# zju3dv/RelightableAvatar

Hardware: AMD Instinct MI355X
Metric: rays_per_sec (higher is better)
Workload: dtype f16

## Files before the change

### relightableavatar_amd/csrc/ra_api.cpp

```cpp
#include "ra_ctx.hpp"
#include <cmath>
#include <map>
#include <mutex>
#include <vector>

#include <cstring>
#include <cstdio>
#include <cstdlib>

static thread_local std::string g_err;
void ra_set_error(const std::string& msg) { g_err = msg; }

#define RA_CHECK(cond, msg)          \
    do {                             \
        if (!(cond)) {               \
            ra_set_error(msg);       \
            return 1;                \
        }                            \
    } while (0)

int DevBuf::ensure(size_t need) {
    if (need <= bytes && p) return 0;
    if (need == 0) need = 16;
    if (p) { hipDeviceSynchronize(); hipFree(p); p = nullptr; bytes = 0; }
// ... 313 lines not shown

void k3_launch(ra_ctx* c, const MlpIO& io, int n, hipStream_t s, int grid_slots = 0) {
    if (c->cfg.mlp_f16) launch_mlp_sdf_stream_f16(c->host.geo, c->sarena.p, c->sarena_pairs.p, c->barena.as<float>(), c->fr, io, n, s, grid_slots);
    else launch_mlp_sdf_stream_bf16(c->host.geo, c->sarena.p, c->sarena_pairs.p, c->barena.as<float>(), c->fr, io, n, s, grid_slots);
}

enum { Q_OTHER = 0, Q_SURFACE = 1 };
bool precise(const ra_ctx* c, int what) { return c->cfg.trace_precision >= 2 || (c->cfg.trace_precision == 1 && what == Q_SURFACE); }
constexpr int KEY_LIGHTS_MAX = 48;
bool key_tier(const ra_ctx* c) { return c->cfg.trace_precision == 1 && c->cfg.key_light_share > 0.f && c->n_lights > 0; }
int key_mask_from(ra_ctx* c, const float* probe, int ph, int pw, hipStream_t s) {
    if (c->key_external) return 0;
    c->key_valid = false;
    if (!key_tier(c) || !probe) return 0;
    if (c->key_mask.ensure((size_t)c->n_lights) || c->key_share.ensure((size_t)c->n_lights * sizeof(float))) return 1;
    launch_key_lights(probe, 1, ph, pw, c->light_dir.as<float>(), c->light_area.as<float>(), c->n_lights, c->cfg.key_light_share, KEY_LIGHTS_MAX, 0,
                      c->key_share.as<float>(), c->key_mask.as<unsigned char>(), s);
    c->key_valid = true;
    return 0;
}

void fine_level(ra_ctx* c, const MlpIO& io, int n, bool comp, hipStream_t s, int hint = -1) {
    const int nv = variant_size(n, hint);
    if (comp) {
        Timer t(c, s, 3);
        launch_mlp_sdf_comp(c->host.geo, c->sarena_c.p, c->barena.as<float>(), c->fr, io, nv, s, c->k3cc_ok, grid_size(n, nv));
    } else {
        Timer t(c, s, k3_waves(nv) == 8 ? 0 : 2);
        k3_launch(c, io, nv, s, grid_size(n, nv));
    }
}

int hdq_pass(ra_ctx* c, const RaySet& rs, int n, float th, int smooth, float* sdf, hipStream_t s, int what = Q_OTHER,
             const unsigned char* key = nullptr, int n_key = 0) {
    if (n <= 0) return 0;
    int err = 0;
    int* fine_idx = c->buf<int>("fine_idx", n, &err);
    float* bpts = c->buf<float>("fine_bpts", (size_t)n * 3, &err);
    if (err) return 1;
    HdqOut out{};
    out.sdf = sdf; out.fine_count = next_fine_counter(c, s); out.fine_idx = fine_idx; out.bpts = bpts;
    const int hint = fine_hint(c, c->fc_next - 1);
    int hint2 = -1;
    if (key && n_key > 0) {
        out.key = key;
        out.fine_idx2 = c->buf<int>("fine_idx_k", n_key, &err);
        out.bpts2 = c->buf<float>("fine_bpts_k", (size_t)n_key * 3, &err);
        if (err) return 1;
        out.fine_count2 = next_fine_counter(c, s);
        hint2 = fine_hint(c, c->fc_next - 1);
    }
    out.counters = dcnt(c);
    launch_hdq_coarse(c->fr, rs, n, th, c->cfg.blend_radius, out, s, c->cfg.use_geodesic_filter != 0);
    MlpIO io{};
    io.bpts = bpts; io.idx = fine_idx; io.count = out.fine_count; io.sdf = sdf; io.dist_th = th; io.smooth = smooth;
    io.resd_limit = c->cfg.resd_limit; io.counters = dcnt(c);
    fine_level(c, io, n, precise(c, what), s, hint);
    if (out.key) {
        io.bpts = out.bpts2; io.idx = out.fine_idx2; io.count = out.fine_count2;
        fine_level(c, io, n_key, true, s, hint2);
    }
    return 0;
}

int full_query(ra_ctx* c, FullIO io, int n, hipStream_t s) {
    const bool gated = c->gate && n > 65536;
    if (gated && c->gate->armed) RA_HIP(hipStreamWaitEvent(s, c->gate->done, 0));
    struct Release {
        ra_ctx* c; hipStream_t s; bool on;
        ~Release() { if (on) { hipEventRecord(c->gate->done, s); c->gate->armed = true; } }
    } release{c, s, gated};
    Timer t(c, s, 1);
    const int batch = c->cfg.k4_batch_slots > 0 ? c->cfg.k4_batch_slots : (1 << 20);
    const int cap = n < batch ? n : batch;
    int err = 0;
    char* tape = c->buf<char>("k4_tape", mlp_full_rev_tape_bytes(cap), &err);
    if (err) {
        ra_set_error("full query: no device memory for the activation tape (" + std::to_string(mlp_full_rev_tape_bytes(cap) >> 20) +
                     " MB): lower cfg.k4_batch_slots / cfg.volume_chunk_rays");
        return 1;
    }
    const bool f16w = c->cfg.mlp_f16 != 0;
    for (int s0 = 0; s0 < n; s0 += cap) {
        io.slot0 = s0;
        io.slot_cap = n - s0 < cap ? n - s0 : cap;
        if (f16w) {
// ... 189 lines not shown
    g.near_offset = near_offset; g.L = L; g.no_visibility = no_visibility; g.local_visibility = local_visibility;
    g.split_wide_groups = split_wide_groups ? 1 : 0;
    g.lvis = lvis; g.ldot = ldot;
    const bool traced = !(no_visibility || local_visibility);
    if (traced) {
        g.ray_pix = c->buf<int>("lv_pix", NR, &err);
        g.ray_light = c->buf<int>("lv_light", NR, &err);
        g.ray_slot = c->buf<int>("lv_slot", NR, &err);
        g.near_ = c->buf<float>("lv_near", NR, &err);
        g.far_ = c->buf<float>("lv_far", NR, &err);
    }
    g.ray_count = icnt(c, CNT_RAYS);
    TraceState sh{};
    float* ssdf = nullptr;
    if (traced) {
        sh = alloc_trace(c, "sh_", (int)NR, shadow.soft_shadow != 0, &err);
        ssdf = c->buf<float>("sh_sdf", NR, &err);
    }
    const bool keyed = traced && key_tier(c) && c->key_valid;
    const size_t NK = keyed ? (size_t)P * (size_t)(L < KEY_LIGHTS_MAX ? L : KEY_LIGHTS_MAX) : 0;
    if (err) return 1;
    if (c->gate && c->gate->armed) RA_HIP(hipStreamWaitEvent(s, c->gate->done, 0));
    launch_shadow_gen(g, P, s, c->cnt_zero);
    c->cnt_zero = false;
    if (traced) {
        sh.near_ = g.near_; sh.far_ = g.far_; sh.tan_i = c->light_sharp.as<float>(); sh.light = g.ray_light;
        launch_trace_init(sh, (int)NR, g.ray_count, shadow, s);
        RaySet r2{};
        r2.mode = 2; r2.o = surf; r2.t = sh.t; r2.pix = g.ray_pix; r2.light = g.ray_light; r2.ldir = c->light_dir.as<float>();
        r2.n_dev = g.ray_count;
        r2.skip = c->cfg.query_skip ? sh.stuck : nullptr;
        r2.nn_hint = c->buf<int>("lv_nn", NR * 3, &err);
        if (err) return 1;
        for (int it = 0; it < shadow.iters; ++it) {
            r2.hint_valid = it > 0;
            r2.hint_src = it == 0 ? pix_nn : nullptr;
            r2.hint_src_index = it == 0 ? g.ray_pix : nullptr;
            if (hdq_pass(c, r2, (int)NR, shadow.dist_th, 1, ssdf, s, Q_OTHER, keyed ? c->key_mask.as<unsigned char>() : nullptr, (int)NK)) return 1;
            launch_trace_update(sh, ssdf, (int)NR, g.ray_count, it, shadow, s);
        }
        launch_shadow_scatter(sh.occ, g.ray_slot, g.ray_count, (int)NR, lvis, s);
        launch_accumulate(g.ray_count, &dcnt(c)->n_shadow_rays, s);
    }
    if (c->gate) { RA_HIP(hipEventRecord(c->gate->done, s)); c->gate->armed = true; }
    *lvis_out = lvis;
    *ldot_out = ldot;
    return 0;
}

int ra_debug_key_lights(ra_ctx* c, unsigned char* key_dev, float* share_dev, void* stream) {
    RA_CHECK(c && key_dev && share_dev, "ra_debug_key_lights: null argument");
    RA_CHECK(c->key_valid && c->n_lights > 0, "ra_debug_key_lights: no key lights have been computed (ra_set_key_probes, or a render call with a probe)");
    RA_HIP(hipSetDevice(c->device));
    RA_HIP(hipMemcpyAsync(key_dev, c->key_mask.p, (size_t)c->n_lights, hipMemcpyDeviceToDevice, (hipStream_t)stream));
    RA_HIP(hipMemcpyAsync(share_dev, c->key_share.p, (size_t)c->n_lights * sizeof(float), hipMemcpyDeviceToDevice, (hipStream_t)stream));
    return 0;
}

int ra_begin_render(ra_ctx* c) {
    RA_CHECK(c, "ra_begin_render: null ctx");
    c->call_no = 0;
    return 0;
}

int ra_set_key_probes(ra_ctx* c, const float* probes, int n, int ph, int pw, int accumulate, void* stream) {
    RA_CHECK(c && n >= 0 && (n == 0 || (probes && ph > 0 && pw > 0)), "ra_set_key_probes: bad arguments");
    if (n == 0) { c->key_external = false; c->key_valid = false; return 0; }
    RA_CHECK(c->have_weights && c->n_lights > 0, "ra_set_key_probes: needs the relight network's light set (ra_finalize_weights)");
    RA_HIP(hipSetDevice(c->device));
    const bool acc = accumulate && c->key_external && c->key_valid;
    c->key_external = true;
    if (!key_tier(c)) { c->key_valid = false; return 0; }
    if (c->key_mask.ensure((size_t)c->n_lights) || c->key_share.ensure((size_t)c->n_lights * sizeof(float))) return 1;
    launch_key_lights(probes, n, ph, pw, c->light_dir.as<float>(), c->light_area.as<float>(), c->n_lights, c->cfg.key_light_share, KEY_LIGHTS_MAX,
// ... 759 lines not shown
```

### relightableavatar_amd/csrc/ra_hdq.hip

```cpp
#include "ra_kernels.hpp"
#include <type_traits>
#include <cstdlib>

namespace {

constexpr int KNN_THREADS = 256;

#ifdef RA_COARSE_TS
__device__ long long ra_coarse_ts[64 * 64 * 16 * 8];
extern "C" int ra_coarse_read_timestamps(long long* out) { return (int)hipMemcpyFromSymbol(out, HIP_SYMBOL(ra_coarse_ts), sizeof(ra_coarse_ts)); }
#define RA_CSTAMP(k) do { if (tsp) { __builtin_amdgcn_sched_barrier(0); if ((threadIdx.x & 63) == 0) tsp[k] = __builtin_readcyclecounter(); __builtin_amdgcn_sched_barrier(0); } } while (0)
#else
#define RA_CSTAMP(k) do { } while (0)
#endif
constexpr int VT = 2048;

__device__ __forceinline__ void inv3d(const float R[9], float M[9]) {
    M[0] = R[4] * R[8] - R[7] * R[5];
    M[3] = -R[3] * R[8] + R[6] * R[5];
    M[6] = R[3] * R[7] - R[6] * R[4];
    M[1] = -R[1] * R[8] + R[7] * R[2];
    M[4] = R[0] * R[8] - R[6] * R[2];
    M[7] = -R[0] * R[7] + R[6] * R[1];
    M[2] = R[1] * R[5] - R[4] * R[2];
    M[5] = -R[0] * R[5] + R[3] * R[2];
    M[8] = R[0] * R[4] - R[3] * R[1];
    const float D = R[0] * M[0] + R[1] * M[3] + R[2] * M[6];
    const float inv = 1.f / (D + 1e-8f);
#pragma unroll
    for (int i = 0; i < 9; ++i) M[i] *= inv;
}

__device__ __forceinline__ float sgn(float x) { return (x > 0.f) ? 1.f : ((x < 0.f) ? -1.f : 0.f); }
// ... 167 lines not shown
    }
}

template <int K>
__device__ __forceinline__ float row_bcast(float v) {
    return __int_as_float(__builtin_amdgcn_update_dpp(0, __float_as_int(v), 0x150 + K, 0xf, 0xf, false));
}

__device__ __forceinline__ float box_dist2(const float p[3], float lx, float ly, float lz, float hx, float hy, float hz) {
    const float dx = fmaxf(fmaxf(lx - p[0], p[0] - hx), 0.f);
    const float dy = fmaxf(fmaxf(ly - p[1], p[1] - hy), 0.f);
    const float dz = fmaxf(fmaxf(lz - p[2], p[2] - hz), 0.f);
    return dx * dx + dy * dy + dz * dz;
}

__device__ __forceinline__ float dist2(float dx, float dy, float dz) { return __fmaf_rn(dz, dz, __fmaf_rn(dx, dx, dy * dy)); }

__device__ __forceinline__ void knn_insert(float d, int id, float& d0, float& d1, float& d2, int& i0, int& i1, int& i2, bool dedup = false) {
    if (__builtin_expect(__ballot(d <= d2) == 0ull, 1)) return;
    bool fresh = true;
    if (dedup) fresh = (id != i0) & (id != i1) & (id != i2);
    const bool c2 = fresh && (d < d2 || (d == d2 && id < i2));
    const bool c1 = fresh && (d < d1 || (d == d1 && id < i1));
    const bool c0 = fresh && (d < d0 || (d == d0 && id < i0));
    const float nd2 = c1 ? d1 : (c2 ? d : d2);
    const int ni2 = c1 ? i1 : (c2 ? id : i2);
    const float nd1 = c0 ? d0 : (c1 ? d : d1);
    const int ni1 = c0 ? i0 : (c1 ? id : i1);
    d0 = c0 ? d : d0;
    i0 = c0 ? id : i0;
    d1 = nd1; i1 = ni1; d2 = nd2; i2 = ni2;
}

__device__ __forceinline__ void ray_point(const RaySet& rs, int i, float x[3]) {
    if (rs.mode == 0) {
        x[0] = rs.x[3 * i]; x[1] = rs.x[3 * i + 1]; x[2] = rs.x[3 * i + 2];
    } else if (rs.mode == 1) {
        const float t = rs.t[i];
        x[0] = rs.o[3 * i] + t * rs.d[3 * i];
        x[1] = rs.o[3 * i + 1] + t * rs.d[3 * i + 1];
        x[2] = rs.o[3 * i + 2] + t * rs.d[3 * i + 2];
    } else {
        const float t = rs.t[i];
        const int p = rs.pix[i], l = rs.light[i];
        x[0] = rs.o[3 * p] + t * rs.ldir[3 * l];
        x[1] = rs.o[3 * p + 1] + t * rs.ldir[3 * l + 1];
        x[2] = rs.o[3 * p + 2] + t * rs.ldir[3 * l + 2];
    }
}

template <bool BVH, int SPLIT, bool HINT = false>
__global__ __launch_bounds__(SPLIT == 1 ? KNN_THREADS : 64 * SPLIT) void hdq_coarse_kernel(FrameState fr, RaySet rs, int n_launch, float th, float inv2r2,
                                                                  HdqOut out, int dbg) {
    static_assert(SPLIT == 1 || (BVH && SPLIT >= 2 && SPLIT <= 16), "SPLIT > 1: the workgroup is SPLIT waves on the same 64 queries");
    constexpr int NT = SPLIT == 1 ? KNN_THREADS : 64 * SPLIT;
    __shared__ __attribute__((aligned(16))) unsigned char smem[BVH ? 16 : VT * 16];
#ifdef RA_COARSE_TS
    long long* tsp = blockIdx.x < 64 ? ra_coarse_ts + ((((dbg >> 8) & 63) * 64 + blockIdx.x) * 16 + (threadIdx.x >> 6)) * 8 : nullptr;
    dbg &= 255;
    if (tsp && (threadIdx.x & 63) == 0) { tsp[1] = tsp[2] = tsp[3] = tsp[4] = tsp[5] = tsp[6] = tsp[7] = 0; }
    RA_CSTAMP(0);
#endif
    const int n = rs.n_dev ? min(*rs.n_dev, n_launch) : n_launch;
    const int base = blockIdx.x * (SPLIT == 1 ? KNN_THREADS : 64);
    if (base >= n) return;
    if (blockIdx.x == 0 && threadIdx.x == 0 && out.counters) atomicAdd(&out.counters->n_coarse, (unsigned long long)n);
    const int i = base + (SPLIT == 1 ? threadIdx.x : (threadIdx.x & 63));
    const bool live_q = i < n && !(rs.skip && rs.skip[i < n ? i : 0]);
    bool live = live_q;
    if (__syncthreads_count(live_q) == 0) return;
    float x[3] = {0.f, 0.f, 0.f};
    if (live) ray_point(rs, i, x);
    const float xt[3] = {x[0] - fr.Th[0], x[1] - fr.Th[1], x[2] - fr.Th[2]};
    float p[3];
#pragma unroll
    for (int c = 0; c < 3; ++c) p[c] = xt[0] * fr.R[c] + xt[1] * fr.R[3 + c] + xt[2] * fr.R[6 + c];

    RA_CSTAMP(1);
    float d0 = 3.0e38f, d1 = 3.0e38f, d2 = 3.0e38f;
    int i0 = 0, i1 = 0, i2 = 0;
    if (dbg & 1) { d0 = 1e-4f; d1 = 2e-4f; d2 = 3e-4f; i0 = 0; i1 = 1; i2 = 2; }
    else if (BVH) {
        const int nl = fr.bvh_leaves, ns = fr.bvh_supers;
        if (!live) { d0 = d1 = d2 = -1.f; }
        const unsigned long long lm = __ballot(live);
        const int first = lm ? __ffsll((long long)lm) - 1 : 0;
        const int lane = threadIdx.x & 63;
        typedef float f2 __attribute__((ext_vector_type(2)));
        const f2 px2 = {p[0], p[0]}, py2 = {p[1], p[1]}, pz2 = {p[2], p[2]};
        constexpr bool hinted = HINT;
#ifdef RA_COARSE_TS
        int n_rare = 0;
#endif
        typedef float f8 __attribute__((ext_vector_type(8)));
        typedef float f4 __attribute__((ext_vector_type(4)));
        typedef int i4 __attribute__((ext_vector_type(4)));
        auto soa8 = [&](int off) __attribute__((always_inline)) { return *(const f8 __attribute__((address_space(4)))*)(fr.bvh_soa + off); };
        auto soa_id4 = [&](int off) __attribute__((always_inline)) { return *(const i4 __attribute__((address_space(4)))*)(fr.bvh_soa + off); };
        auto box4 = [&](int off) __attribute__((always_inline)) {
            return *(const f4 __attribute__((address_space(4)))*)(reinterpret_cast<const float*>(fr.bvh_sbox) + off);
        };
        auto box1 = [&](int off) __attribute__((always_inline)) { return reinterpret_cast<const float*>(fr.bvh_sbox)[off]; };
        auto scan_leaf = [&](int l) __attribute__((always_inline)) {
            const int L = l * (4 * BVH_LEAF);
            f8 cx = soa8(L), cy = soa8(L + BVH_LEAF), cz = soa8(L + 2 * BVH_LEAF), nx = cx, ny = cy, nz = cz;
// ... 242 lines not shown
#pragma unroll
        for (int e = 0; e < 24; ++e) out.dbg_mats[(size_t)i * 24 + e] = M[e];
    }
}

}

void launch_vert_blend(const float* weights, const float* A, const float* big_A, int n_verts, int n_bones, float* vertA,
                       hipStream_t s) {
    hipLaunchKernelGGL(vert_blend_kernel, dim3((n_verts + 255) / 256), dim3(256), 0, s, weights, A, big_A, n_verts, n_bones, vertA);
}

void launch_pack_verts(const float* pverts, int n_verts, float4* out, hipStream_t s) {
    hipLaunchKernelGGL(pack_verts_kernel, dim3((n_verts + 255) / 256), dim3(256), 0, s, pverts, n_verts, out);
}

void launch_fold_bias(const float* W, int ld, int col0, int ncond, const float* cond, const float* bias, float* out,
                      hipStream_t s) {
    hipLaunchKernelGGL(fold_bias_kernel, dim3(64), dim3(256), 0, s, W, ld, col0, ncond, cond, bias, out);
}

int bvh_leaf_count(int n_verts) {
    if (n_verts > BVH_MAXN) return 0;
    return (n_verts + BVH_LEAF - 1) / BVH_LEAF;
}
int bvh_super_count(int n_leaves) { return (n_leaves + BVH_FAN - 1) / BVH_FAN; }

void launch_bvh_build(const float4* pverts4, int n_verts, int* order, float* leaves, float4* sbox, int n_leaves, int n_supers, hipStream_t s) {
    hipLaunchKernelGGL(bvh_rank_kernel, dim3((n_verts + 63) / 64), dim3(BVH_THREADS), 0, s, pverts4, n_verts, order);
    hipLaunchKernelGGL(bvh_boxes_kernel, dim3(1), dim3(BVH_THREADS), 0, s, pverts4, order, n_verts, leaves, sbox, n_leaves, n_supers);
}

void launch_hdq_coarse(const FrameState& fr, const RaySet& rs, int n, float th, float blend_radius, const HdqOut& out,
                       hipStream_t s, bool geodesic) {
    if (n <= 0) return;
    const float inv2r2 = 1.f / (2.f * blend_radius * blend_radius);
    const dim3 grid((n + KNN_THREADS - 1) / KNN_THREADS);
    int dbg = 0, probe = 0, split_max = 196608;
#ifdef RA_TESTING
    static const int e_dbg = getenv("RA_COARSE_DBG") ? atoi(getenv("RA_COARSE_DBG")) : 0;
    static const int e_probe = getenv("RA_COARSE_PROBE") ? atoi(getenv("RA_COARSE_PROBE")) : 0;
    static const int e_split = getenv("RA_COARSE_SPLIT_MAX") ? atoi(getenv("RA_COARSE_SPLIT_MAX")) : 196608;
    dbg = e_dbg; probe = e_probe; split_max = e_split;
#endif
    if (!geodesic) dbg |= 32;
#ifdef RA_COARSE_TS
    static int launch_no = 0;
    dbg |= (launch_no++ & 63) << 8;
#endif
    const bool hint = (rs.nn_hint != nullptr && rs.hint_valid != 0) || rs.hint_src != nullptr;
    for (int pass = probe ? 0 : 1; pass < 2; ++pass) {
        const int d = pass == 0 ? probe : dbg;
        if (fr.bvh_leaves > 0 && n <= split_max)
        {
            const int groups = (n + 63) / 64;
            if (hint) {
                if (n <= split_max / 8) hipLaunchKernelGGL((hdq_coarse_kernel<true, 16, true>), dim3(groups), dim3(1024), 0, s, fr, rs, n, th, inv2r2, out, d);
                else if (n <= split_max / 2) hipLaunchKernelGGL((hdq_coarse_kernel<true, 8, true>), dim3(groups), dim3(512), 0, s, fr, rs, n, th, inv2r2, out, d);
                else hipLaunchKernelGGL((hdq_coarse_kernel<true, 4, true>), dim3(groups), dim3(256), 0, s, fr, rs, n, th, inv2r2, out, d);
            } else {
                if (n <= split_max / 8) hipLaunchKernelGGL((hdq_coarse_kernel<true, 16>), dim3(groups), dim3(1024), 0, s, fr, rs, n, th, inv2r2, out, d);
                else if (n <= split_max / 2) hipLaunchKernelGGL((hdq_coarse_kernel<true, 8>), dim3(groups), dim3(512), 0, s, fr, rs, n, th, inv2r2, out, d);
                else hipLaunchKernelGGL((hdq_coarse_kernel<true, 4>), dim3(groups), dim3(256), 0, s, fr, rs, n, th, inv2r2, out, d);
            }
        }
        else if (fr.bvh_leaves > 0 && hint) hipLaunchKernelGGL((hdq_coarse_kernel<true, 1, true>), grid, dim3(KNN_THREADS), 0, s, fr, rs, n, th, inv2r2, out, d);
        else if (fr.bvh_leaves > 0) hipLaunchKernelGGL((hdq_coarse_kernel<true, 1>), grid, dim3(KNN_THREADS), 0, s, fr, rs, n, th, inv2r2, out, d);
        else hipLaunchKernelGGL((hdq_coarse_kernel<false, 1>), grid, dim3(KNN_THREADS), 0, s, fr, rs, n, th, inv2r2, out, d);
        if (pass == 0) hipMemsetAsync(out.fine_count, 0, sizeof(int), s);
    }
}
```

### relightableavatar_amd/csrc/ra_kernels.hpp

```cpp
#pragma once
#include "ra_common.hpp"

struct RaySet {
    int mode;
    const float* x;
    const float* o;
    const float* d;
    const float* t;
    const int* pix;
    const int* light;
    const float* ldir;
    const int* n_dev;
    const unsigned char* skip;
    int* nn_hint;
    int hint_valid;
    const int* hint_src;
    const int* hint_src_index;
};

struct HdqOut {
    float* sdf;
    int* fine_count;
    int* fine_idx;
    float* bpts;
    float* mats;
    const unsigned char* key;
    int* fine_count2;
    int* fine_idx2;
    float* bpts2;
    float* raw_zero;
    int raw_C;
    float* dbg_sdf_batch;
    int* dbg_nn_batch;
    float* dbg_d2;
    float* dbg_tpts;
    float* dbg_bpts;
    float* dbg_mats;
    DevCounters* counters;
};

void launch_vert_blend(const float* weights, const float* A, const float* big_A, int n_verts, int n_bones, float* vertA,
                       hipStream_t s);
void launch_pack_verts(const float* pverts, int n_verts, float4* out, hipStream_t s);
void launch_fold_bias(const float* W, int ld, int col0, int ncond, const float* cond, const float* bias, float* out,
                      hipStream_t s);
void launch_bvh_build(const float4* pverts4, int n_verts, int* order, float* leaves, float4* sbox, int n_leaves, int n_supers, hipStream_t s);
int bvh_leaf_count(int n_verts);
int bvh_super_count(int n_leaves);
void launch_hdq_coarse(const FrameState& fr, const RaySet& rs, int n, float th, float blend_radius, const HdqOut& out,
                       hipStream_t s, bool geodesic = true);

struct TraceState {
    float *t, *d0, *dt, *st, *ot, *cd, *occ, *off, *rlx;
    const float *near_, *far_;
    const float* tan_i;
    const int* light;
    unsigned char* stuck;
};
void launch_trace_init(const TraceState& ts, int n, const int* n_dev, const ra_trace_params& p, hipStream_t s);

void launch_trace_update(const TraceState& ts, const float* sdf, int n, const int* n_dev, int iter,
                         const ra_trace_params& p, hipStream_t s);

void launch_surface_finish(const float* ray_o, const float* ray_d, const float* st, const float* occ, int P, float* surf,
                           float* depth, float* acc, int* hit_idx, int* hit_count, hipStream_t s, int* slot_of_ray = nullptr,
                           bool counter_is_zero = false);
void launch_slot_index(const int* hit_idx, const int* hit_count, int P, int* slot_of_ray, hipStream_t s);
struct MapJob { const float* src; float* dst; int C; int premul; int src_full; };
constexpr int RA_MAX_MAP_JOBS = 16;
struct EmitMaps { MapJob job[RA_MAX_MAP_JOBS]; long long end[RA_MAX_MAP_JOBS]; int n_jobs; const int* slot_of_ray; const float* acc; const int* perm; int P; };
void launch_emit_maps(const EmitMaps& m, hipStream_t s);
void launch_surface_samples(const float* surf, const float* ray_d, const int* hit_idx, const int* hit_count, int P, int S,
                            float range, float* x, float* v, int* n_out, hipStream_t s);
struct SurfaceMaps {
    float *cpts, *bpts, *resd, *norm, *albedo, *rough, *rgb;
    float* valbedo;
};
void launch_surface_composite(const float* raw, int C, int S, const int* hit_count, int P, int relight, const ra_config& cfg,
                              const SurfaceMaps& m, hipStream_t s);

constexpr int RA_MAX_BOXES = 32;
struct ShadowGen {
    const float* surf;
    const float* norm;
    const float* acc;
    const int* hit_idx;
    const int* hit_count;
    const float* ldir;
    float bbox[6];
    int n_boxes;
    float boxes[RA_MAX_BOXES][6];
    int box_start[RA_MAX_BOXES + 1];
    const int* perm;
    float near_offset;
    int L;
    int no_visibility, local_visibility;
    int split_wide_groups;
    float* lvis;
    float* ldot;
    int* ray_pix;
    int* ray_light;
    int* ray_slot;
    float *near_, *far_;
    int* ray_count;
};
void launch_key_lights(const float* probes, int n, int ph, int pw, const float* ldir, const float* area, int L, float share, int kmax,
                       int accumulate, float* smax, unsigned char* key, hipStream_t s);
void launch_gather_shard_rays(const long long* idx, int n, const float* ro, const float* rd, const float* nr, const float* fr, float* so, float* sd,
                              float* sn, float* sf, hipStream_t s);
void launch_scatter_rows(const float* src, const long long* src_idx, const long long* dst_idx, long long n, int C, float* dst, hipStream_t s);
void launch_shadow_gen(const ShadowGen& g, int P, hipStream_t s, bool counter_is_zero = false);
void launch_debug_aabb(const float* o, const float* d, int n, const float* bbox6, float* nr, float* fr, hipStream_t s);
void launch_debug_brdf(const float* p2l, const float* p2c, const float* nrm, const float* alb, const float* rough, int L, int N, const ra_config& cfg,
                       float* out, hipStream_t s);
size_t sort_hits_temp_bytes(int P);
int launch_sort_hits(const float* surf, const float* acc, int P, const float* bbox_min, unsigned* keys_in, unsigned* keys_out,
                     int* vals_in, int* hit_idx_out, void* temp, size_t temp_bytes, hipStream_t s);
void launch_shadow_scatter(const float* occ, const int* ray_slot, const int* ray_count, int max_rays, float* lvis, hipStream_t s);

struct ShadeIn {
    const float* ray_o;
    const float* surf;
    const int* idx;
    const int* count;
    int n;
    const float *norm, *albedo, *rough;
    const float *lvis, *ldot;
    const float *light_xyz, *light_area;
    int L;
    const float* probes;
    int n_probes, ph, pw;
    int want_spec;
    float *rgb, *shade, *spec;
};
void launch_shade(const ShadeIn& in, const ra_config& cfg, hipStream_t s);

void launch_scatter_maps(const int* hit_idx, const int* hit_count, int P, int premultiply, const float* acc_full,
                         const float* src, int C, float* dst, int src_full, const int* perm, hipStream_t s);
int launch_sort_rays(const float* ro, const float* rd, const float* nr, const float* fr, int P, const float* bbox_min, unsigned* keys_in,
                     unsigned* keys_out, int* vals_in, int* perm, void* temp, size_t temp_bytes, float* so, float* sd, float* sn, float* sf,
                     hipStream_t s, float near_min = -3.0e38f, float far_max = 3.0e38f);
void launch_accumulate(const int* count, unsigned long long* dst, hipStream_t s);

void launch_volume_samples(const float* ray_o, const float* ray_d, const float* near_, const float* far_, int P, int S,
                           float* x, float* v, hipStream_t s);
void launch_volume_composite(const float* raw, int C, const float* near_, const float* far_, int P, int S, float bg,
                             const ra_render_out& out, const int* perm, hipStream_t s);
void launch_fill(float* p, size_t n, float v, hipStream_t s);
void launch_iota(int* idx, int n, int* count, hipStream_t s);
void launch_bigpose_compose(const float* mats, const float* d2, int n, float blend_radius, const float* R, const float* Th, int invert, float* out,
                            hipStream_t s);
// ... 67 lines not shown
```

### relightableavatar_amd/csrc/ra_trace.hip

```cpp
#include "ra_kernels.hpp"
#include <hipcub/hipcub.hpp>

namespace {

constexpr int TPB = 256;
constexpr float PI_F = 3.14159265358979323846f;

__device__ __forceinline__ int live_count(const int* n_dev, int n) { return n_dev ? min(*n_dev, n) : n; }

__device__ __forceinline__ float linspace01(int s, int S) {
    if (S == 1) return 0.f;
    const float step = 1.f / (float)(S - 1);
    return (s < S / 2) ? (float)s * step : 1.f - (float)(S - 1 - s) * step;
}

__global__ void trace_init_kernel(TraceState ts, int n_launch, const int* n_dev, float offset, float relax) {
    const int i = blockIdx.x * TPB + threadIdx.x;
    if (i >= live_count(n_dev, n_launch)) return;
    const float nr = ts.near_[i], fr = ts.far_[i];
    ts.t[i] = nr;
    ts.d0[i] = 1e9f;
    ts.occ[i] = 1.f;
    if (ts.stuck) ts.stuck[i] = 0;
    if (ts.dt) ts.dt[i] = 1e9f;
    if (ts.st) ts.st[i] = fr;
    if (ts.ot) ts.ot[i] = fr;
    if (ts.cd) ts.cd[i] = 1e9f;
    if (ts.off) ts.off[i] = offset;
    if (ts.rlx) ts.rlx[i] = relax;
}

template <bool SOFT>
__global__ void trace_update_kernel(TraceState ts, const float* __restrict__ sdf, int n_launch, const int* n_dev, int iter,
                                    ra_trace_params p) {
    const int i = blockIdx.x * TPB + threadIdx.x;
    if (i >= live_count(n_dev, n_launch)) return;
    const float d1 = sdf[i];
    const float d0 = ts.d0[i];
    float t = ts.t[i];
    const float t_prev = t;
    float occ = ts.occ[i];
    const float nr = ts.near_[i], fr = ts.far_[i];
    float tan_i = p.tan_i;
    if (SOFT) {
        const float ti = ts.tan_i ? (ts.light ? ts.tan_i[ts.light[i]] : ts.tan_i[i]) : p.tan_i;
        tan_i = p.tan_i_multiplier * ti;
    }
    const float tan2 = (1.f / tan_i) * 2.f;
    float off = ts.off ? ts.off[i] : p.offset;
    float rlx = ts.rlx ? ts.rlx[i] : p.relax;
    float ot = ts.ot ? ts.ot[i] : 0.f;
    if (SOFT && p.clay_book && iter >= p.shadow_skip_iter) {
        const float dx0 = d0 + rlx * d0 + off;
        const float dx1 = d1 + rlx * d1 + off;
        const float dy = (dx1 * dx1) / (2.f * dx0);
        const float dx = (sqrtf(dx1 * dx1 - dy * dy) - off) / (1.f + rlx);
        const float den = fmaxf(fmaxf(t - dy, nr), p.eps);
        const float cls = fmaxf(dx, 0.f) / den / tan2;
        const bool msk = (cls < occ) && (dy < t) && (dx1 > 0.f) && (dx0 > 0.f) && (dx > 0.f) && (dy > 0.f) && (dy < dx0);
        if (msk) { ot = t - dy; occ = cls; }
    }
    if (iter >= p.shadow_skip_iter) {
        const float cls = fmaxf(d1, 0.f) / fmaxf(fmaxf(t, nr), p.eps) / tan2;
        if (cls < occ) { ot = t; occ = cls; }
    }
    if (!SOFT) {
        const float d1u = fabsf(d1), d0u = fabsf(d0);
        float st = ts.st[i], cd = ts.cd[i];
        const float dt = ts.dt[i];
        const float s0 = (d0 > 0.f) ? 1.f : ((d0 < 0.f) ? -1.f : 0.f);
        const float s1 = (d1 > 0.f) ? 1.f : ((d1 < 0.f) ? -1.f : 0.f);
        if (s0 != s1) {
            st = t - dt * fminf(fmaxf(d1u / (d0u + d1u + p.eps), 0.f), 1.f);
            off = 0.f;
            rlx = 0.f;
        }
        if (d1u < cd) { cd = d1u; st = t; }
        ts.st[i] = st;
        ts.cd[i] = cd;
        ts.off[i] = off;
        ts.rlx[i] = rlx;
    }
    const float dtn = d1 + rlx * d1 + off;
    t = t + dtn;
    t = fminf(t, fr);
    t = fmaxf(t, nr);
    if (ts.dt) ts.dt[i] = dtn;
    ts.t[i] = t;
    if (ts.stuck) ts.stuck[i] = (t == t_prev || (SOFT && occ == 0.f)) ? 1 : 0;
    ts.d0[i] = d1;
    ts.occ[i] = occ;
    if (ts.ot) ts.ot[i] = ot;
}

__global__ void surface_finish_kernel(const float* __restrict__ ro, const float* __restrict__ rd, const float* __restrict__ st,
                                      const float* __restrict__ occ, int P, float* __restrict__ surf, float* __restrict__ depth,
                                      float* __restrict__ acc, int* __restrict__ hit_idx, int* __restrict__ hit_count, int* __restrict__ slot_of_ray) {
    const int i = blockIdx.x * TPB + threadIdx.x;
    bool hit = false;
    if (i < P) {
        if (slot_of_ray) slot_of_ray[i] = -1;
        const float s = st[i];
        const float sx = ro[3 * i] + s * rd[3 * i], sy = ro[3 * i + 1] + s * rd[3 * i + 1], sz = ro[3 * i + 2] + s * rd[3 * i + 2];
        surf[3 * i] = sx; surf[3 * i + 1] = sy; surf[3 * i + 2] = sz;
        depth[i] = (sx - ro[3 * i]) / rd[3 * i];
        const float a = 1.f - occ[i];
        acc[i] = a;
        hit = a > 0.f;
    }
    const unsigned long long m = __ballot(hit);
    if (m == 0ull) return;
    const int lane = threadIdx.x & 63;
    int base = 0;
    if (lane == 0) base = atomicAdd(hit_count, __popcll(m));
    base = __shfl(base, 0);
    if (hit) hit_idx[base + __popcll(m & ((1ull << lane) - 1ull))] = i;
}

__device__ __forceinline__ unsigned expand10t(unsigned v) {
    v = (v * 0x00010001u) & 0xFF0000FFu;
    v = (v * 0x00000101u) & 0x0F00F00Fu;
    v = (v * 0x00000011u) & 0xC30C30C3u;
    v = (v * 0x00000005u) & 0x49249249u;
    return v;
}
// ... 268 lines not shown
    const int gbase = cnt[0][NL];
#pragma unroll
    for (int round = 0; round < ROUNDS; ++round) {
        const int ll = round * (TPB / 64) + wv;
        const bool trace = (tmask >> round) & 1u;
        const unsigned long long m = __ballot(trace);
        if (trace) {
            const int hf = lane >> 5;
            const unsigned mh = hf ? (unsigned)(m >> 32) : (unsigned)m;
            const int s = gbase + cnt[hf][ll] + __popc(mh & ((1u << (lane & 31)) - 1u));
            const int l = lc * SG_LIGHTS + ll;
            g.ray_pix[s] = r;
            g.ray_light[s] = l;
            g.ray_slot[s] = h * g.L + l;
            g.near_[s] = nrv[round];
            g.far_[s] = frv[round];
        }
    }
    const int col = threadIdx.x & (SG_LIGHTS - 1), l = lc * SG_LIGHTS + col;
    for (int row = threadIdx.x / SG_LIGHTS; row < 64; row += TPB / SG_LIGHTS) {
        const int hh = grp * 64 + row;
        if (hh < nh && l < g.L) {
            g.ldot[(size_t)hh * g.L + l] = t_ldot[row][col];
            g.lvis[(size_t)hh * g.L + l] = t_lvis[row][col];
        }
    }
}

__global__ void shadow_scatter_kernel(const float* __restrict__ occ, const int* __restrict__ ray_slot, const int* __restrict__ ray_count,
                                      int max_rays, float* __restrict__ lvis) {
    const int i = blockIdx.x * TPB + threadIdx.x;
    if (i >= min(*ray_count, max_rays)) return;
    lvis[ray_slot[i]] = occ[i];
}

__device__ __forceinline__ float safe_div(float& a, float& b) {
    const float eps = 1e-8f;
    if (a < eps && a >= 0.f) a = eps;
    if (a > -eps && a <= 0.f) a = -eps;
    if (b < eps && b >= 0.f) b = eps;
    if (b > -eps && b <= 0.f) b = -eps;
    float d = a / b;
    if (d != d) d = 0.f;
    if (isinf(d)) d = 0.f;
    return fminf(fmaxf(d, -1e10f), 1e10f);
}

__device__ __forceinline__ void fnormalize(float v[3]) {
    const float n = fmaxf(sqrtf(v[0] * v[0] + v[1] * v[1] + v[2] * v[2]), 1e-7f);
    v[0] /= n; v[1] /= n; v[2] /= n;
}

__device__ __forceinline__ void sample_probe(const float* __restrict__ img, int H, int W, const float d[3], float out[3]) {
    const float theta = acosf(d[2]) - 1e-6f;
    const float phi = atan2f(d[1], d[0]);
    const float qy = (theta / PI_F) * 2.f - 1.f;
    const float qx = -phi / PI_F;
    float ix = ((qx + 1.f) * W - 1.f) * 0.5f;
    float iy = ((qy + 1.f) * H - 1.f) * 0.5f;
    ix = fminf(fmaxf(ix, 0.f), (float)(W - 1));
    iy = fminf(fmaxf(iy, 0.f), (float)(H - 1));
    const float fx = floorf(ix), fy = floorf(iy);
    const int x0 = (int)fx, y0 = (int)fy, x1 = x0 + 1, y1 = y0 + 1;
    const float wx1 = ix - fx, wy1 = iy - fy, wx0 = 1.f - wx1, wy0 = 1.f - wy1;
    out[0] = out[1] = out[2] = 0.f;
    auto add = [&](int xx, int yy, float w) {
// ... 850 lines not shown
    size_t bytes = 0;
    hipcub::DeviceSelect::Flagged(nullptr, bytes, hipcub::CountingInputIterator<int>(0), (const unsigned char*)nullptr, (int*)nullptr, (int*)nullptr, n);
    return bytes;
}

int launch_gen_rays(const RayCam& cam, unsigned char* mask, int* pix_idx, int* count_dev, void* temp, size_t temp_bytes,
                    float* ray_o, float* ray_d, float* near, float* far, hipStream_t s) {
    const int n = cam.H * cam.W;
    if (n <= 0) { hipMemsetAsync(count_dev, 0, sizeof(int), s); return 0; }
    hipLaunchKernelGGL(ray_mask_kernel, grid_for(n), dim3(TPB), 0, s, cam, mask);
    if (hipcub::DeviceSelect::Flagged(temp, temp_bytes, hipcub::CountingInputIterator<int>(0), mask, pix_idx, count_dev, n, s) != hipSuccess) return 1;
    hipLaunchKernelGGL(ray_emit_kernel, grid_for(n), dim3(TPB), 0, s, cam, pix_idx, count_dev, ray_o, ray_d, near, far);
    return 0;
}

size_t sort_hits_temp_bytes(int P) {
    size_t bytes = 0;
    hipcub::DeviceRadixSort::SortPairs(nullptr, bytes, (const unsigned*)nullptr, (unsigned*)nullptr, (const int*)nullptr, (int*)nullptr, P);
    return bytes;
}

int launch_sort_hits(const float* surf, const float* acc, int P, const float* bbox_min, unsigned* keys_in, unsigned* keys_out,
                     int* vals_in, int* hit_idx_out, void* temp, size_t temp_bytes, hipStream_t s) {
    if (P <= 0) return 0;
    hipLaunchKernelGGL(hit_keys_kernel, grid_for(P), dim3(TPB), 0, s, surf, acc, P, bbox_min[0], bbox_min[1], bbox_min[2], keys_in, vals_in);
    return hipcub::DeviceRadixSort::SortPairs(temp, temp_bytes, keys_in, keys_out, vals_in, hit_idx_out, P, 0, 32, s) == hipSuccess ? 0 : 1;
}

void launch_shadow_scatter(const float* occ, const int* ray_slot, const int* ray_count, int max_rays, float* lvis, hipStream_t s) {
    if (max_rays <= 0) return;
    hipLaunchKernelGGL(shadow_scatter_kernel, grid_for(max_rays), dim3(TPB), 0, s, occ, ray_slot, ray_count, max_rays, lvis);
}

void launch_shade(const ShadeIn& in, const ra_config& cfg, hipStream_t s) {
    if (in.n <= 0) return;
    hipLaunchKernelGGL(shade_kernel, grid_for((long long)in.n * 64), dim3(TPB), 0, s, in, cfg);
}

void launch_scatter_maps(const int* hit_idx, const int* hit_count, int P, int premultiply, const float* acc_full, const float* src,
                         int C, float* dst, int src_full, const int* perm, hipStream_t s) {
    if (P <= 0) return;
    hipLaunchKernelGGL(scatter_maps_kernel, grid_for((long long)P * C), dim3(TPB), 0, s, hit_idx, hit_count, premultiply, acc_full, src, C, dst, src_full, perm);
}

int launch_sort_rays(const float* ro, const float* rd, const float* nr, const float* fr, int P, const float* bbox_min, unsigned* keys_in,
                     unsigned* keys_out, int* vals_in, int* perm, void* temp, size_t temp_bytes, float* so, float* sd, float* sn, float* sf,
                     hipStream_t s, float near_min, float far_max) {
    if (P <= 0) return 0;
    float* origin_dev = nullptr;
    if (!bbox_min) {
        origin_dev = reinterpret_cast<float*>(keys_out);
        hipLaunchKernelGGL(entry_min_kernel, dim3(1), dim3(1024), 0, s, ro, rd, nr, P, origin_dev);
    }
    hipLaunchKernelGGL(ray_keys_kernel, grid_for(P), dim3(TPB), 0, s, ro, rd, nr, P, bbox_min ? bbox_min[0] : 0.f, bbox_min ? bbox_min[1] : 0.f,
                       bbox_min ? bbox_min[2] : 0.f, origin_dev, keys_in, vals_in);
    if (hipcub::DeviceRadixSort::SortPairs(temp, temp_bytes, keys_in, keys_out, vals_in, perm, P, 0, 32, s) != hipSuccess) return 1;
    hipLaunchKernelGGL(gather_rays_kernel, grid_for(P), dim3(TPB), 0, s, perm, P, ro, rd, nr, fr, so, sd, sn, sf, near_min, far_max);
    return 0;
}

void launch_gather_shard_rays(const long long* idx, int n, const float* ro, const float* rd, const float* nr, const float* fr, float* so, float* sd,
                              float* sn, float* sf, hipStream_t s) {
    if (n <= 0) return;
    hipLaunchKernelGGL(gather_shard_rays_kernel, grid_for(n), dim3(TPB), 0, s, idx, n, ro, rd, nr, fr, so, sd, sn, sf);
}

// ... 90 lines not shown
```

Baseline: 9.017 million.

## Fuse soft-shadow trace update into next hdq coarse kernel and final scatter

For soft shadows, the per-iteration trace_update kernel is folded into the following hinted BVH coarse query kernel: each thread computes the trace step in registers, stores the state, and uses the new t directly for its ray point. The last iteration's update is merged into a new shadow_finish kernel that writes lvis directly. This removes one launch and one global round-trip of the trace state per iteration. In exchange there are more kernel template variants, more registers in the coarse kernel, and a fallback path when the BVH/hint conditions are not met.

```diff
diff --git a/relightableavatar_amd/csrc/ra_api.cpp b/relightableavatar_amd/csrc/ra_api.cpp
--- a/relightableavatar_amd/csrc/ra_api.cpp
+++ b/relightableavatar_amd/csrc/ra_api.cpp
@@ -369,7 +369,7 @@
 }
 
 int hdq_pass(ra_ctx* c, const RaySet& rs, int n, float th, int smooth, float* sdf, hipStream_t s, int what = Q_OTHER,
-             const unsigned char* key = nullptr, int n_key = 0) {
+             const unsigned char* key = nullptr, int n_key = 0, const TraceFuse* fuse = nullptr) {
     if (n <= 0) return 0;
     int err = 0;
     int* fine_idx = c->buf<int>("fine_idx", n, &err);
@@ -388,7 +388,7 @@
         hint2 = fine_hint(c, c->fc_next - 1);
     }
     out.counters = dcnt(c);
-    launch_hdq_coarse(c->fr, rs, n, th, c->cfg.blend_radius, out, s, c->cfg.use_geodesic_filter != 0);
+    launch_hdq_coarse(c->fr, rs, n, th, c->cfg.blend_radius, out, s, c->cfg.use_geodesic_filter != 0, fuse);
     MlpIO io{};
     io.bpts = bpts; io.idx = fine_idx; io.count = out.fine_count; io.sdf = sdf; io.dist_th = th; io.smooth = smooth;
     io.resd_limit = c->cfg.resd_limit; io.counters = dcnt(c);
@@ -644,14 +644,21 @@
         r2.skip = c->cfg.query_skip ? sh.stuck : nullptr;
         r2.nn_hint = c->buf<int>("lv_nn", NR * 3, &err);
         if (err) return 1;
+        static const bool fuse_env = !(getenv("RA_SHADOW_UPDATE_FUSED") && atoi(getenv("RA_SHADOW_UPDATE_FUSED")) == 0);
+        const bool fused = fuse_env && shadow.soft_shadow != 0 && shadow.iters > 0;
+        TraceFuse fu{};
+        fu.ts = sh; fu.sdf = ssdf; fu.p = shadow;
         for (int it = 0; it < shadow.iters; ++it) {
             r2.hint_valid = it > 0;
             r2.hint_src = it == 0 ? pix_nn : nullptr;
             r2.hint_src_index = it == 0 ? g.ray_pix : nullptr;
-            if (hdq_pass(c, r2, (int)NR, shadow.dist_th, 1, ssdf, s, Q_OTHER, keyed ? c->key_mask.as<unsigned char>() : nullptr, (int)NK)) return 1;
-            launch_trace_update(sh, ssdf, (int)NR, g.ray_count, it, shadow, s);
+            fu.iter = it - 1;
+            if (hdq_pass(c, r2, (int)NR, shadow.dist_th, 1, ssdf, s, Q_OTHER, keyed ? c->key_mask.as<unsigned char>() : nullptr, (int)NK,
+                         fused && it > 0 ? &fu : nullptr)) return 1;
+            if (!fused) launch_trace_update(sh, ssdf, (int)NR, g.ray_count, it, shadow, s);
         }
-        launch_shadow_scatter(sh.occ, g.ray_slot, g.ray_count, (int)NR, lvis, s);
+        if (fused) launch_shadow_finish(sh, ssdf, g.ray_slot, g.ray_count, (int)NR, shadow.iters - 1, shadow, lvis, s);
+        else launch_shadow_scatter(sh.occ, g.ray_slot, g.ray_count, (int)NR, lvis, s);
         launch_accumulate(g.ray_count, &dcnt(c)->n_shadow_rays, s);
     }
     if (c->gate) { RA_HIP(hipEventRecord(c->gate->done, s)); c->gate->armed = true; }
diff --git a/relightableavatar_amd/csrc/ra_hdq.hip b/relightableavatar_amd/csrc/ra_hdq.hip
--- a/relightableavatar_amd/csrc/ra_hdq.hip
+++ b/relightableavatar_amd/csrc/ra_hdq.hip
@@ -1,4 +1,5 @@
 #include "ra_kernels.hpp"
+#include "ra_trace_step.hpp"
 #include <type_traits>
 #include <cstdlib>
 
@@ -232,16 +233,16 @@
     d1 = nd1; i1 = ni1; d2 = nd2; i2 = ni2;
 }
 
-__device__ __forceinline__ void ray_point(const RaySet& rs, int i, float x[3]) {
+__device__ __forceinline__ void ray_point(const RaySet& rs, int i, float x[3], const float* t_reg = nullptr) {
     if (rs.mode == 0) {
         x[0] = rs.x[3 * i]; x[1] = rs.x[3 * i + 1]; x[2] = rs.x[3 * i + 2];
     } else if (rs.mode == 1) {
-        const float t = rs.t[i];
+        const float t = t_reg ? *t_reg : rs.t[i];
         x[0] = rs.o[3 * i] + t * rs.d[3 * i];
         x[1] = rs.o[3 * i + 1] + t * rs.d[3 * i + 1];
         x[2] = rs.o[3 * i + 2] + t * rs.d[3 * i + 2];
     } else {
-        const float t = rs.t[i];
+        const float t = t_reg ? *t_reg : rs.t[i];
         const int p = rs.pix[i], l = rs.light[i];
         x[0] = rs.o[3 * p] + t * rs.ldir[3 * l];
         x[1] = rs.o[3 * p + 1] + t * rs.ldir[3 * l + 1];
@@ -249,10 +250,11 @@
     }
 }
 
-template <bool BVH, int SPLIT, bool HINT = false>
+template <bool BVH, int SPLIT, bool HINT = false, bool UPD = false>
 __global__ __launch_bounds__(SPLIT == 1 ? KNN_THREADS : 64 * SPLIT) void hdq_coarse_kernel(FrameState fr, RaySet rs, int n_launch, float th, float inv2r2,
-                                                                  HdqOut out, int dbg) {
+                                                                  HdqOut out, int dbg, TraceFuse fu) {
     static_assert(SPLIT == 1 || (BVH && SPLIT >= 2 && SPLIT <= 16), "SPLIT > 1: the workgroup is SPLIT waves on the same 64 queries");
+    static_assert(!UPD || (BVH && HINT), "UPD: a variant of the hinted BVH kernels");
     constexpr int NT = SPLIT == 1 ? KNN_THREADS : 64 * SPLIT;
     __shared__ __attribute__((aligned(16))) unsigned char smem[BVH ? 16 : VT * 16];
 #ifdef RA_COARSE_TS
@@ -266,11 +268,15 @@
     if (base >= n) return;
     if (blockIdx.x == 0 && threadIdx.x == 0 && out.counters) atomicAdd(&out.counters->n_coarse, (unsigned long long)n);
     const int i = base + (SPLIT == 1 ? threadIdx.x : (threadIdx.x & 63));
-    const bool live_q = i < n && !(rs.skip && rs.skip[i < n ? i : 0]);
+    TraceStep step{};
+    if (UPD && i < n) step = trace_step<true>(fu.ts, fu.sdf, i, fu.iter, fu.p, false);
+    const bool live_q = i < n && (UPD ? !(rs.skip && step.stuck) : !(rs.skip && rs.skip[i < n ? i : 0]));
     bool live = live_q;
-    if (__syncthreads_count(live_q) == 0) return;
+    const int n_live = __syncthreads_count(live_q);
+    if (UPD && i < n && (SPLIT == 1 || threadIdx.x < 64)) trace_step_store(fu.ts, i, step);
+    if (n_live == 0) return;
     float x[3] = {0.f, 0.f, 0.f};
-    if (live) ray_point(rs, i, x);
+    if (live) ray_point(rs, i, x, UPD ? &step.t : nullptr);
     const float xt[3] = {x[0] - fr.Th[0], x[1] - fr.Th[1], x[2] - fr.Th[2]};
     float p[3];
 #pragma unroll
@@ -579,7 +585,7 @@
 }
 
 void launch_hdq_coarse(const FrameState& fr, const RaySet& rs, int n, float th, float blend_radius, const HdqOut& out,
-                       hipStream_t s, bool geodesic) {
+                       hipStream_t s, bool geodesic, const TraceFuse* fuse) {
     if (n <= 0) return;
     const float inv2r2 = 1.f / (2.f * blend_radius * blend_radius);
     const dim3 grid((n + KNN_THREADS - 1) / KNN_THREADS);
@@ -596,24 +602,34 @@
     dbg |= (launch_no++ & 63) << 8;
 #endif
     const bool hint = (rs.nn_hint != nullptr && rs.hint_valid != 0) || rs.hint_src != nullptr;
+    if (fuse && !(fr.bvh_leaves > 0 && hint && rs.mode == 2 && fuse->p.soft_shadow && !probe)) {
+        launch_trace_update(fuse->ts, fuse->sdf, n, rs.n_dev, fuse->iter, fuse->p, s);
+        fuse = nullptr;
+    }
+    const TraceFuse fu = fuse ? *fuse : TraceFuse{};
     for (int pass = probe ? 0 : 1; pass < 2; ++pass) {
         const int d = pass == 0 ? probe : dbg;
         if (fr.bvh_leaves > 0 && n <= split_max)
         {
             const int groups = (n + 63) / 64;
-            if (hint) {
-                if (n <= split_max / 8) hipLaunchKernelGGL((hdq_coarse_kernel<true, 16, true>), dim3(groups), dim3(1024), 0, s, fr, rs, n, th, inv2r2, out, d);
-                else if (n <= split_max / 2) hipLaunchKernelGGL((hdq_coarse_kernel<true, 8, true>), dim3(groups), dim3(512), 0, s, fr, rs, n, th, inv2r2, out, d);
-                else hipLaunchKernelGGL((hdq_coarse_kernel<true, 4, true>), dim3(groups), dim3(256), 0, s, fr, rs, n, th, inv2r2, out, d);
+            if (fuse) {
+                if (n <= split_max / 8) hipLaunchKernelGGL((hdq_coarse_kernel<true, 16, true, true>), dim3(groups), dim3(1024), 0, s, fr, rs, n, th, inv2r2, out, d, fu);
+                else if (n <= split_max / 2) hipLaunchKernelGGL((hdq_coarse_kernel<true, 8, true, true>), dim3(groups), dim3(512), 0, s, fr, rs, n, th, inv2r2, out, d, fu);
+                else hipLaunchKernelGGL((hdq_coarse_kernel<true, 4, true, true>), dim3(groups), dim3(256), 0, s, fr, rs, n, th, inv2r2, out, d, fu);
+            } else if (hint) {
+                if (n <= split_max / 8) hipLaunchKernelGGL((hdq_coarse_kernel<true, 16, true>), dim3(groups), dim3(1024), 0, s, fr, rs, n, th, inv2r2, out, d, fu);
+                else if (n <= split_max / 2) hipLaunchKernelGGL((hdq_coarse_kernel<true, 8, true>), dim3(groups), dim3(512), 0, s, fr, rs, n, th, inv2r2, out, d, fu);
+                else hipLaunchKernelGGL((hdq_coarse_kernel<true, 4, true>), dim3(groups), dim3(256), 0, s, fr, rs, n, th, inv2r2, out, d, fu);
             } else {
-                if (n <= split_max / 8) hipLaunchKernelGGL((hdq_coarse_kernel<true, 16>), dim3(groups), dim3(1024), 0, s, fr, rs, n, th, inv2r2, out, d);
-                else if (n <= split_max / 2) hipLaunchKernelGGL((hdq_coarse_kernel<true, 8>), dim3(groups), dim3(512), 0, s, fr, rs, n, th, inv2r2, out, d);
-                else hipLaunchKernelGGL((hdq_coarse_kernel<true, 4>), dim3(groups), dim3(256), 0, s, fr, rs, n, th, inv2r2, out, d);
-            }
-        }
-        else if (fr.bvh_leaves > 0 && hint) hipLaunchKernelGGL((hdq_coarse_kernel<true, 1, true>), grid, dim3(KNN_THREADS), 0, s, fr, rs, n, th, inv2r2, out, d);
-        else if (fr.bvh_leaves > 0) hipLaunchKernelGGL((hdq_coarse_kernel<true, 1>), grid, dim3(KNN_THREADS), 0, s, fr, rs, n, th, inv2r2, out, d);
-        else hipLaunchKernelGGL((hdq_coarse_kernel<false, 1>), grid, dim3(KNN_THREADS), 0, s, fr, rs, n, th, inv2r2, out, d);
+                if (n <= split_max / 8) hipLaunchKernelGGL((hdq_coarse_kernel<true, 16>), dim3(groups), dim3(1024), 0, s, fr, rs, n, th, inv2r2, out, d, fu);
+                else if (n <= split_max / 2) hipLaunchKernelGGL((hdq_coarse_kernel<true, 8>), dim3(groups), dim3(512), 0, s, fr, rs, n, th, inv2r2, out, d, fu);
+                else hipLaunchKernelGGL((hdq_coarse_kernel<true, 4>), dim3(groups), dim3(256), 0, s, fr, rs, n, th, inv2r2, out, d, fu);
+            }
+        }
+        else if (fuse) hipLaunchKernelGGL((hdq_coarse_kernel<true, 1, true, true>), grid, dim3(KNN_THREADS), 0, s, fr, rs, n, th, inv2r2, out, d, fu);
+        else if (fr.bvh_leaves > 0 && hint) hipLaunchKernelGGL((hdq_coarse_kernel<true, 1, true>), grid, dim3(KNN_THREADS), 0, s, fr, rs, n, th, inv2r2, out, d, fu);
+        else if (fr.bvh_leaves > 0) hipLaunchKernelGGL((hdq_coarse_kernel<true, 1>), grid, dim3(KNN_THREADS), 0, s, fr, rs, n, th, inv2r2, out, d, fu);
+        else hipLaunchKernelGGL((hdq_coarse_kernel<false, 1>), grid, dim3(KNN_THREADS), 0, s, fr, rs, n, th, inv2r2, out, d, fu);
         if (pass == 0) hipMemsetAsync(out.fine_count, 0, sizeof(int), s);
     }
 }
diff --git a/relightableavatar_amd/csrc/ra_kernels.hpp b/relightableavatar_amd/csrc/ra_kernels.hpp
--- a/relightableavatar_amd/csrc/ra_kernels.hpp
+++ b/relightableavatar_amd/csrc/ra_kernels.hpp
@@ -47,8 +47,9 @@
 void launch_bvh_build(const float4* pverts4, int n_verts, int* order, float* leaves, float4* sbox, int n_leaves, int n_supers, hipStream_t s);
 int bvh_leaf_count(int n_verts);
 int bvh_super_count(int n_leaves);
+struct TraceFuse;
 void launch_hdq_coarse(const FrameState& fr, const RaySet& rs, int n, float th, float blend_radius, const HdqOut& out,
-                       hipStream_t s, bool geodesic = true);
+                       hipStream_t s, bool geodesic = true, const TraceFuse* fuse = nullptr);
 
 struct TraceState {
     float *t, *d0, *dt, *st, *ot, *cd, *occ, *off, *rlx;
@@ -61,6 +62,13 @@
 
 void launch_trace_update(const TraceState& ts, const float* sdf, int n, const int* n_dev, int iter,
                          const ra_trace_params& p, hipStream_t s);
+
+struct TraceFuse {
+    TraceState ts;
+    const float* sdf;
+    int iter;
+    ra_trace_params p;
+};
 
 void launch_surface_finish(const float* ray_o, const float* ray_d, const float* st, const float* occ, int P, float* surf,
                            float* depth, float* acc, int* hit_idx, int* hit_count, hipStream_t s, int* slot_of_ray = nullptr,
@@ -117,6 +125,8 @@
 int launch_sort_hits(const float* surf, const float* acc, int P, const float* bbox_min, unsigned* keys_in, unsigned* keys_out,
                      int* vals_in, int* hit_idx_out, void* temp, size_t temp_bytes, hipStream_t s);
 void launch_shadow_scatter(const float* occ, const int* ray_slot, const int* ray_count, int max_rays, float* lvis, hipStream_t s);
+void launch_shadow_finish(const TraceState& ts, const float* sdf, const int* ray_slot, const int* ray_count, int max_rays, int iter,
+                          const ra_trace_params& p, float* lvis, hipStream_t s);
 
 struct ShadeIn {
     const float* ray_o;
diff --git a/relightableavatar_amd/csrc/ra_trace.hip b/relightableavatar_amd/csrc/ra_trace.hip
--- a/relightableavatar_amd/csrc/ra_trace.hip
+++ b/relightableavatar_amd/csrc/ra_trace.hip
@@ -1,4 +1,5 @@
 #include "ra_kernels.hpp"
+#include "ra_trace_step.hpp"
 #include <hipcub/hipcub.hpp>
 
 namespace {
@@ -35,62 +36,7 @@
                                     ra_trace_params p) {
     const int i = blockIdx.x * TPB + threadIdx.x;
     if (i >= live_count(n_dev, n_launch)) return;
-    const float d1 = sdf[i];
-    const float d0 = ts.d0[i];
-    float t = ts.t[i];
-    const float t_prev = t;
-    float occ = ts.occ[i];
-    const float nr = ts.near_[i], fr = ts.far_[i];
-    float tan_i = p.tan_i;
-    if (SOFT) {
-        const float ti = ts.tan_i ? (ts.light ? ts.tan_i[ts.light[i]] : ts.tan_i[i]) : p.tan_i;
-        tan_i = p.tan_i_multiplier * ti;
-    }
-    const float tan2 = (1.f / tan_i) * 2.f;
-    float off = ts.off ? ts.off[i] : p.offset;
-    float rlx = ts.rlx ? ts.rlx[i] : p.relax;
-    float ot = ts.ot ? ts.ot[i] : 0.f;
-    if (SOFT && p.clay_book && iter >= p.shadow_skip_iter) {
-        const float dx0 = d0 + rlx * d0 + off;
-        const float dx1 = d1 + rlx * d1 + off;
-        const float dy = (dx1 * dx1) / (2.f * dx0);
-        const float dx = (sqrtf(dx1 * dx1 - dy * dy) - off) / (1.f + rlx);
-        const float den = fmaxf(fmaxf(t - dy, nr), p.eps);
-        const float cls = fmaxf(dx, 0.f) / den / tan2;
-        const bool msk = (cls < occ) && (dy < t) && (dx1 > 0.f) && (dx0 > 0.f) && (dx > 0.f) && (dy > 0.f) && (dy < dx0);
-        if (msk) { ot = t - dy; occ = cls; }
-    }
-    if (iter >= p.shadow_skip_iter) {
-        const float cls = fmaxf(d1, 0.f) / fmaxf(fmaxf(t, nr), p.eps) / tan2;
-        if (cls < occ) { ot = t; occ = cls; }
-    }
-    if (!SOFT) {
-        const float d1u = fabsf(d1), d0u = fabsf(d0);
-        float st = ts.st[i], cd = ts.cd[i];
-        const float dt = ts.dt[i];
-        const float s0 = (d0 > 0.f) ? 1.f : ((d0 < 0.f) ? -1.f : 0.f);
-        const float s1 = (d1 > 0.f) ? 1.f : ((d1 < 0.f) ? -1.f : 0.f);
-        if (s0 != s1) {
-            st = t - dt * fminf(fmaxf(d1u / (d0u + d1u + p.eps), 0.f), 1.f);
-            off = 0.f;
-            rlx = 0.f;
-        }
-        if (d1u < cd) { cd = d1u; st = t; }
-        ts.st[i] = st;
-        ts.cd[i] = cd;
-        ts.off[i] = off;
-        ts.rlx[i] = rlx;
-    }
-    const float dtn = d1 + rlx * d1 + off;
-    t = t + dtn;
-    t = fminf(t, fr);
-    t = fmaxf(t, nr);
-    if (ts.dt) ts.dt[i] = dtn;
-    ts.t[i] = t;
-    if (ts.stuck) ts.stuck[i] = (t == t_prev || (SOFT && occ == 0.f)) ? 1 : 0;
-    ts.d0[i] = d1;
-    ts.occ[i] = occ;
-    if (ts.ot) ts.ot[i] = ot;
+    trace_step<SOFT>(ts, sdf, i, iter, p, true);
 }
 
 __global__ void surface_finish_kernel(const float* __restrict__ ro, const float* __restrict__ rd, const float* __restrict__ st,
@@ -425,6 +371,13 @@
     const int i = blockIdx.x * TPB + threadIdx.x;
     if (i >= min(*ray_count, max_rays)) return;
     lvis[ray_slot[i]] = occ[i];
+}
+
+__global__ void shadow_finish_kernel(TraceState ts, const float* __restrict__ sdf, const int* __restrict__ ray_slot, const int* __restrict__ ray_count,
+                                     int max_rays, int iter, ra_trace_params p, float* __restrict__ lvis) {
+    const int i = blockIdx.x * TPB + threadIdx.x;
+    if (i >= min(*ray_count, max_rays)) return;
+    lvis[ray_slot[i]] = trace_step<true>(ts, sdf, i, iter, p, false).occ;
 }
 
 __device__ __forceinline__ float safe_div(float& a, float& b) {
@@ -1341,6 +1294,12 @@
     hipLaunchKernelGGL(shadow_scatter_kernel, grid_for(max_rays), dim3(TPB), 0, s, occ, ray_slot, ray_count, max_rays, lvis);
 }
 
+void launch_shadow_finish(const TraceState& ts, const float* sdf, const int* ray_slot, const int* ray_count, int max_rays, int iter,
+                          const ra_trace_params& p, float* lvis, hipStream_t s) {
+    if (max_rays <= 0) return;
+    hipLaunchKernelGGL(shadow_finish_kernel, grid_for(max_rays), dim3(TPB), 0, s, ts, sdf, ray_slot, ray_count, max_rays, iter, p, lvis);
+}
+
 void launch_shade(const ShadeIn& in, const ra_config& cfg, hipStream_t s) {
     if (in.n <= 0) return;
     hipLaunchKernelGGL(shade_kernel, grid_for((long long)in.n * 64), dim3(TPB), 0, s, in, cfg);
diff --git a/relightableavatar_amd/csrc/ra_trace_step.hpp b/relightableavatar_amd/csrc/ra_trace_step.hpp
--- /dev/null
+++ b/relightableavatar_amd/csrc/ra_trace_step.hpp
@@ -0,0 +1,82 @@
+#pragma once
+#include "ra_kernels.hpp"
+
+struct TraceStep {
+    float t, d0, occ, ot;
+    unsigned char stuck;
+};
+
+__device__ __forceinline__ void trace_step_store(const TraceState& ts, int i, const TraceStep& r) {
+    ts.t[i] = r.t;
+    if (ts.stuck) ts.stuck[i] = r.stuck;
+    ts.d0[i] = r.d0;
+    ts.occ[i] = r.occ;
+    if (ts.ot) ts.ot[i] = r.ot;
+}
+
+template <bool SOFT>
+__device__ __forceinline__ TraceStep trace_step(const TraceState& ts, const float* __restrict__ sdf, int i, int iter, const ra_trace_params& p,
+                                                bool store) {
+#pragma clang fp contract(off)
+    const float d1 = sdf[i];
+    const float d0 = ts.d0[i];
+    float t = ts.t[i];
+    const float t_prev = t;
+    float occ = ts.occ[i];
+    const float nr = ts.near_[i], fr = ts.far_[i];
+    float tan_i = p.tan_i;
+    if (SOFT) {
+        const float ti = ts.tan_i ? (ts.light ? ts.tan_i[ts.light[i]] : ts.tan_i[i]) : p.tan_i;
+        tan_i = p.tan_i_multiplier * ti;
+    }
+    const float tan2 = (1.f / tan_i) * 2.f;
+    float off = ts.off ? ts.off[i] : p.offset;
+    float rlx = ts.rlx ? ts.rlx[i] : p.relax;
+    float ot = ts.ot ? ts.ot[i] : 0.f;
+    if (SOFT && p.clay_book && iter >= p.shadow_skip_iter) {
+        const float dx0 = __fmaf_rn(rlx, d0, d0) + off;
+        const float dx1 = __fmaf_rn(rlx, d1, d1) + off;
+        const float sq1 = dx1 * dx1;
+        const float dy = sq1 / (2.f * dx0);
+        const float dx = (sqrtf(__fmaf_rn(-dy, dy, sq1)) - off) / (1.f + rlx);
+        const float den = fmaxf(fmaxf(t - dy, nr), p.eps);
+        const float cls = fmaxf(dx, 0.f) / den / tan2;
+        const bool msk = (cls < occ) && (dy < t) && (dx1 > 0.f) && (dx0 > 0.f) && (dx > 0.f) && (dy > 0.f) && (dy < dx0);
+        if (msk) { ot = t - dy; occ = cls; }
+    }
+    if (iter >= p.shadow_skip_iter) {
+        const float cls = fmaxf(d1, 0.f) / fmaxf(fmaxf(t, nr), p.eps) / tan2;
+        if (cls < occ) { ot = t; occ = cls; }
+    }
+    if (!SOFT) {
+        const float d1u = fabsf(d1), d0u = fabsf(d0);
+        float st = ts.st[i], cd = ts.cd[i];
+        const float dt = ts.dt[i];
+        const float s0 = (d0 > 0.f) ? 1.f : ((d0 < 0.f) ? -1.f : 0.f);
+        const float s1 = (d1 > 0.f) ? 1.f : ((d1 < 0.f) ? -1.f : 0.f);
+        if (s0 != s1) {
+            st = __fmaf_rn(-fminf(fmaxf(d1u / (d0u + d1u + p.eps), 0.f), 1.f), dt, t);
+            off = 0.f;
+            rlx = 0.f;
+        }
+        if (d1u < cd) { cd = d1u; st = t; }
+        if (store) {
+            ts.st[i] = st;
+            ts.cd[i] = cd;
+            ts.off[i] = off;
+            ts.rlx[i] = rlx;
+        }
+    }
+    const float dtn = __fmaf_rn(rlx, d1, d1) + off;
+    t = t + dtn;
+    t = fminf(t, fr);
+    t = fmaxf(t, nr);
+    TraceStep r;
+    r.t = t; r.d0 = d1; r.occ = occ; r.ot = ot;
+    r.stuck = (t == t_prev || (SOFT && occ == 0.f)) ? 1 : 0;
+    if (store) {
+        if (ts.dt) ts.dt[i] = dtn;
+        trace_step_store(ts, i, r);
+    }
+    return r;
+}
```

Result: no change. 9.067 million (median of 6 runs) (+0.6%).
